# yondonfu/ai-rtc-agent

Hardware: NVIDIA H100
Metric: frames/sec at 512x512 SD-Turbo img2img (1-step, stream-batch 1) (higher is better)
Workload: dtype f16

## Files before the change

### ai-rtc-agent_b200/csrc/attention.cu

```cuda
#include "attention.cuh"

#include <cudaTypedefs.h>
#include <math.h>
#include <string.h>

#include "igemm.cuh"
#include "launch.cuh"
#include "ptx.cuh"
#include "wgmma.cuh"

namespace b2 {

constexpr int AT_BQ = 128;
constexpr int AT_STAGES = 3;
constexpr int AT_CONS = 256;
constexpr int AT_THREADS = AT_CONS + 32;

__device__ __forceinline__ float ex2_approx(float x) {
    float y;
    asm volatile("ex2.approx.ftz.f32 %0, %1;" : "=f"(y) : "f"(x));
    return y;
}

__device__ __forceinline__ uint32_t pack_half2(float a, float b) {
    const __half2 h = __floats2half2_rn(a, b);
    return *reinterpret_cast<const uint32_t*>(&h);
}

struct AttnParams {
    CUtensorMap tmq, tmk, tmv;
    __half* out;
    int ldo;
    int sq, skv, heads, d_real;
    long k_bstride, vt_bstride;
    float scale_log2;
};

struct AttnIpParams : AttnParams {
    CUtensorMap tmk_ip, tmv_ip;
    const int* n_ip;
};

template <int DA, int BKV, bool IP = false>
__global__ void __launch_bounds__(AT_THREADS, 1) attn_kernel(const __grid_constant__ std::conditional_t<IP, AttnIpParams, AttnParams> p) {
    constexpr int DP = DA * 64;
    constexpr int NST = AT_STAGES;
    constexpr int KVA = BKV / 64;
    constexpr uint32_t Q_BYTES = DA * AT_BQ * 128;
    constexpr uint32_t K_BYTES = DA * BKV * 128;
    constexpr uint32_t V_BYTES = KVA * DP * 128;
    constexpr uint32_t STAGE_BYTES = K_BYTES + V_BYTES;

    extern __shared__ __align__(1024) uint8_t smem[];
    uint8_t* sQ = smem;
    uint8_t* sKV = sQ + Q_BYTES;
    uint64_t* bars = reinterpret_cast<uint64_t*>(sKV + NST * STAGE_BYTES);
    uint64_t* q_full = bars;
    uint64_t* k_full = bars + 1;
    uint64_t* k_empty = k_full + NST;
    uint64_t* v_full = k_empty + NST;
    uint64_t* v_empty = v_full + NST;

    const int warp = threadIdx.x >> 5, lane = threadIdx.x & 31;
    const int q0 = blockIdx.x * AT_BQ;
    const int h = blockIdx.y, b = blockIdx.z;
    const int nblk = (p.skv + BKV - 1) / BKV;

    if (threadIdx.x == AT_CONS) {
        if (smem_u32(smem) & 1023u) {
            printf("b2 attn: dynamic smem base not 1024-aligned\n");
            __trap();
        }
        tma_prefetch_desc(&p.tmq);
        tma_prefetch_desc(&p.tmk);
        tma_prefetch_desc(&p.tmv);
        mbar_init(q_full, 1);
        for (int s = 0; s < NST; ++s) {
            mbar_init(&k_full[s], 1);
            mbar_init(&k_empty[s], AT_CONS / 32);
            mbar_init(&v_full[s], 1);
            mbar_init(&v_empty[s], AT_CONS / 32);
        }
        fence_mbar_init();
    }
    __syncthreads();
    pdl_launch_dependents();
    pdl_wait();
    int n_ip = 0;
    if constexpr (IP) n_ip = *p.n_ip;

    if (warp == AT_CONS / 32) {
        if (lane == 0) {
            mbar_expect_tx(q_full, Q_BYTES);
#pragma unroll
            for (int a = 0; a < DA; ++a)
                tma_load_2d(sQ + a * (AT_BQ * 128), &p.tmq, q_full, h * DP + a * 64, b * p.sq + q0);
            auto load_k = [&](int j) {
                const int st = j % NST;
                mbar_wait(&k_empty[st], ((j / NST) & 1) ^ 1);
                uint8_t* sk = sKV + st * STAGE_BYTES;
                mbar_expect_tx(&k_full[st], K_BYTES);
#pragma unroll
                for (int a = 0; a < DA; ++a)
                    tma_load_2d(sk + a * (BKV * 128), &p.tmk, &k_full[st], h * DP + a * 64, (int)(b * p.k_bstride) + j * BKV);
            };
            auto load_v = [&](int j) {
                const int st = j % NST;
                mbar_wait(&v_empty[st], ((j / NST) & 1) ^ 1);
                uint8_t* sv = sKV + st * STAGE_BYTES + K_BYTES;
                mbar_expect_tx(&v_full[st], V_BYTES);
#pragma unroll
                for (int a = 0; a < KVA; ++a)
                    tma_load_2d(sv + a * (DP * 128), &p.tmv, &v_full[st], (int)(b * p.vt_bstride) + j * BKV + a * 64, h * DP);
            };
            auto load_k_ip = [&]() {
                if constexpr (IP) {
                    const int st = nblk % NST;
                    mbar_wait(&k_empty[st], ((nblk / NST) & 1) ^ 1);
                    uint8_t* sk = sKV + st * STAGE_BYTES;
                    mbar_expect_tx(&k_full[st], DA * ATTN_IP_KEYS * 128);
#pragma unroll
                    for (int a = 0; a < DA; ++a)
                        tma_load_2d(sk + a * (ATTN_IP_KEYS * 128), &p.tmk_ip, &k_full[st], h * DP + a * 64, 0);
                }
            };
            auto load_v_ip = [&]() {
                if constexpr (IP) {
                    const int st = nblk % NST;
                    mbar_wait(&v_empty[st], ((nblk / NST) & 1) ^ 1);
                    mbar_expect_tx(&v_full[st], DP * 128);
                    tma_load_2d(sKV + st * STAGE_BYTES + K_BYTES, &p.tmv_ip, &v_full[st], 0, h * DP);
                }
            };
            load_k(0);
            for (int j = 0; j < nblk; ++j) {
                if (j + 1 < nblk) load_k(j + 1);
                else if (n_ip > 0) load_k_ip();
                load_v(j);
            }
            if (n_ip > 0) load_v_ip();
        }
    } else {
        const int wg = warp >> 2;
        const int rq = wg * 64 + (warp & 3) * 16 + (lane >> 2);
        const int q2 = 2 * (lane & 3);
        const uint32_t sq_addr = smem_u32(sQ) + (uint32_t)wg * (64 * 128), skv_addr = smem_u32(sKV);
        float m_run[2] = {-INFINITY, -INFINITY}, l_run[2] = {0.f, 0.f};
        float o[DP / 2];
#pragma unroll
        for (int i = 0; i < DP / 2; ++i) o[i] = 0.f;
        mbar_wait(q_full, 0);
        for (int j = 0; j < nblk; ++j) {
            const int st = j % NST;
            const uint32_t ph = (uint32_t)(j / NST) & 1u;
            const uint32_t sk = skv_addr + st * STAGE_BYTES;
            float s[BKV / 2];
#pragma unroll
            for (int i = 0; i < BKV / 2; ++i) s[i] = 0.f;
            mbar_wait(&k_full[st], ph);
            wgmma_fence_regs(s);
            wgmma_fence();
#pragma unroll
            for (int a = 0; a < DA; ++a) {
                const uint64_t dq = make_kmajor_sw128_desc(sq_addr + a * (AT_BQ * 128));
                const uint64_t dk = make_kmajor_sw128_desc(sk + a * (BKV * 128));
#pragma unroll
                for (int k = 0; k < 4; ++k) Wgmma<BKV>::ss(s, dq + 2 * k, dk + 2 * k, 1u);
            }
            wgmma_commit();
            wgmma_wait<0>();
            wgmma_fence_regs(s);
            if (lane == 0) mbar_arrive(&k_empty[st]);
            const int kv_valid = p.skv - j * BKV;
            float alpha[2], m_new[2];
#pragma unroll
            for (int hr = 0; hr < 2; ++hr) {
                float mx = -INFINITY;
#pragma unroll
                for (int jj = 0; jj < BKV / 8; ++jj)
#pragma unroll
                    for (int u = 0; u < 2; ++u)
                        if (8 * jj + q2 + u < kv_valid) mx = fmaxf(mx, s[4 * jj + 2 * hr + u]);
                mx = fmaxf(mx, __shfl_xor_sync(0xffffffffu, mx, 1));
                mx = fmaxf(mx, __shfl_xor_sync(0xffffffffu, mx, 2));
                m_new[hr] = fmaxf(m_run[hr], mx * p.scale_log2);
                alpha[hr] = ex2_approx(m_run[hr] - m_new[hr]);
            }
            uint32_t pa[BKV / 16][4];
            float rs[2] = {0.f, 0.f};
#pragma unroll
            for (int jj = 0; jj < BKV / 8; ++jj)
#pragma unroll
                for (int hr = 0; hr < 2; ++hr) {
                    float p0 = ex2_approx(s[4 * jj + 2 * hr] * p.scale_log2 - m_new[hr]);
                    float p1 = ex2_approx(s[4 * jj + 2 * hr + 1] * p.scale_log2 - m_new[hr]);
                    if (8 * jj + q2 >= kv_valid) p0 = 0.f;
                    if (8 * jj + q2 + 1 >= kv_valid) p1 = 0.f;
                    rs[hr] += p0 + p1;
                    pa[jj >> 1][(jj & 1) * 2 + hr] = pack_half2(p0, p1);
                }
#pragma unroll
            for (int hr = 0; hr < 2; ++hr) {
                l_run[hr] = l_run[hr] * alpha[hr] + rs[hr];
                m_run[hr] = m_new[hr];
            }
#pragma unroll
            for (int jj = 0; jj < DP / 8; ++jj)
#pragma unroll
                for (int hr = 0; hr < 2; ++hr) {
                    o[4 * jj + 2 * hr] *= alpha[hr];
                    o[4 * jj + 2 * hr + 1] *= alpha[hr];
                }
            const uint32_t sv = sk + K_BYTES;
            mbar_wait(&v_full[st], ph);
            wgmma_fence_regs(o);
            wgmma_fence();
#pragma unroll
            for (int kk = 0; kk < BKV / 16; ++kk) {
                const uint64_t dv = make_kmajor_sw128_desc(sv + (kk >> 2) * (DP * 128)) + 2 * (kk & 3);
                Wgmma<DP>::rs(o, pa[kk], dv, 1u);
            }
            wgmma_commit();
            wgmma_wait<0>();
            wgmma_fence_regs(o);
            if (lane == 0) mbar_arrive(&v_empty[st]);
        }
        if (n_ip > 0) {
            const int st = nblk % NST;
            const uint32_t ph = (uint32_t)(nblk / NST) & 1u;
            const uint32_t sk = skv_addr + st * STAGE_BYTES;
            float s[ATTN_IP_KEYS / 2];
#pragma unroll
            for (int i = 0; i < ATTN_IP_KEYS / 2; ++i) s[i] = 0.f;
            mbar_wait(&k_full[st], ph);
            wgmma_fence_regs(s);
            wgmma_fence();
#pragma unroll
            for (int a = 0; a < DA; ++a) {
                const uint64_t dq = make_kmajor_sw128_desc(sq_addr + a * (AT_BQ * 128));
                const uint64_t dk = make_kmajor_sw128_desc(sk + a * (ATTN_IP_KEYS * 128));
#pragma unroll
                for (int k = 0; k < 4; ++k) Wgmma<ATTN_IP_KEYS>::ss(s, dq + 2 * k, dk + 2 * k, 1u);
            }
            wgmma_commit();
            wgmma_wait<0>();
            wgmma_fence_regs(s);
            float m2[2], f2[2];
#pragma unroll
            for (int hr = 0; hr < 2; ++hr) {
                float mx = -INFINITY;
#pragma unroll
                for (int jj = 0; jj < ATTN_IP_KEYS / 8; ++jj)
#pragma unroll
                    for (int u = 0; u < 2; ++u)
                        if (8 * jj + q2 + u < n_ip) mx = fmaxf(mx, s[4 * jj + 2 * hr + u]);
                mx = fmaxf(mx, __shfl_xor_sync(0xffffffffu, mx, 1));
                mx = fmaxf(mx, __shfl_xor_sync(0xffffffffu, mx, 2));
                m2[hr] = mx * p.scale_log2;
            }
            float p2[ATTN_IP_KEYS / 2];
            float rs[2] = {0.f, 0.f};
#pragma unroll
            for (int jj = 0; jj < ATTN_IP_KEYS / 8; ++jj)
#pragma unroll
                for (int hr = 0; hr < 2; ++hr)
#pragma unroll
                    for (int u = 0; u < 2; ++u) {
                        float e = ex2_approx(s[4 * jj + 2 * hr + u] * p.scale_log2 - m2[hr]);
                        if (8 * jj + q2 + u >= n_ip) e = 0.f;
                        p2[4 * jj + 2 * hr + u] = e;
                        rs[hr] += e;
                    }
#pragma unroll
            for (int hr = 0; hr < 2; ++hr) {
                float l = l_run[hr], l2 = rs[hr];
                l += __shfl_xor_sync(0xffffffffu, l, 1);
                l += __shfl_xor_sync(0xffffffffu, l, 2);
                l2 += __shfl_xor_sync(0xffffffffu, l2, 1);
                l2 += __shfl_xor_sync(0xffffffffu, l2, 2);
                f2[hr] = l / l2;
            }
            uint32_t pa[ATTN_IP_KEYS / 16][4];
#pragma unroll
            for (int jj = 0; jj < ATTN_IP_KEYS / 8; ++jj)
#pragma unroll
                for (int hr = 0; hr < 2; ++hr)
                    pa[jj >> 1][(jj & 1) * 2 + hr] = pack_half2(p2[4 * jj + 2 * hr] * f2[hr], p2[4 * jj + 2 * hr + 1] * f2[hr]);
            const uint32_t sv = sk + K_BYTES;
            mbar_wait(&v_full[st], ph);
            wgmma_fence_regs(o);
            wgmma_fence();
#pragma unroll
            for (int kk = 0; kk < ATTN_IP_KEYS / 16; ++kk) Wgmma<DP>::rs(o, pa[kk], make_kmajor_sw128_desc(sv) + 2 * kk, 1u);
            wgmma_commit();
            wgmma_wait<0>();
            wgmma_fence_regs(o);
        }
#pragma unroll
        for (int hr = 0; hr < 2; ++hr) {
            float l = l_run[hr];
            l += __shfl_xor_sync(0xffffffffu, l, 1);
            l += __shfl_xor_sync(0xffffffffu, l, 2);
            const float inv_l = 1.0f / l;
            const int r = rq + 8 * hr;
            if (q0 + r >= p.sq) continue;
            __half* orow = p.out + ((long)b * p.sq + q0 + r) * p.ldo + h * p.d_real;
#pragma unroll
            for (int jj = 0; jj < DP / 8; ++jj) {
                const int col = 8 * jj + q2;
                if (col < p.d_real)
                    *reinterpret_cast<uint32_t*>(orow + col) = pack_half2(o[4 * jj + 2 * hr] * inv_l, o[4 * jj + 2 * hr + 1] * inv_l);
            }
        }
    }
}

constexpr int A5_D = 512;
constexpr int A5_DS = 128;
constexpr int A5_SLICES = A5_D / A5_DS;
constexpr int A5_BQ = 128;
constexpr int A5_BKV = 32;
constexpr int A5_THREADS = 256;
constexpr int A5_QP = A5_D + 8;
constexpr int A5_VP = A5_BKV + 8;
constexpr size_t A5_Q_ELEMS = (size_t)A5_BQ * A5_QP;
constexpr size_t A5_K_ELEMS = (size_t)A5_BKV * A5_QP;
constexpr size_t A5_V_ELEMS = (size_t)A5_DS * A5_VP;
constexpr size_t A5_SMEM = (A5_Q_ELEMS + 2 * (A5_K_ELEMS + A5_V_ELEMS)) * 2;

struct Attn512Params {
    const __half* q; const __half* k; const __half* vt;
    __half* out;
    int ldq, ldk, ldvt, ldo;
    int sq, skv;
    long k_bstride, vt_bstride;
    float scale_log2;
};

__device__ __forceinline__ void cp_async16(uint32_t dst, const void* src, int src_bytes) {
    asm volatile("cp.async.cg.shared.global [%0], [%1], 16, %2;" ::"r"(dst), "l"(src), "r"(src_bytes) : "memory");
}
__device__ __forceinline__ void cp_async_commit() { asm volatile("cp.async.commit_group;" ::: "memory"); }
template <int N>
__device__ __forceinline__ void cp_async_wait() { asm volatile("cp.async.wait_group %0;" ::"n"(N) : "memory"); }
__device__ __forceinline__ void ldsm_x4(uint32_t addr, uint32_t& r0, uint32_t& r1, uint32_t& r2, uint32_t& r3) {
    asm volatile("ldmatrix.sync.aligned.m8n8.x4.shared.b16 {%0,%1,%2,%3}, [%4];"
                 : "=r"(r0), "=r"(r1), "=r"(r2), "=r"(r3) : "r"(addr));
}
__device__ __forceinline__ void mma16816(float (&d)[4], const uint32_t (&a)[4], uint32_t b0, uint32_t b1) {
    asm volatile("mma.sync.aligned.m16n8k16.row.col.f32.f16.f16.f32 {%0,%1,%2,%3}, {%4,%5,%6,%7}, {%8,%9}, {%0,%1,%2,%3};"
                 : "+f"(d[0]), "+f"(d[1]), "+f"(d[2]), "+f"(d[3])
                 : "r"(a[0]), "r"(a[1]), "r"(a[2]), "r"(a[3]), "r"(b0), "r"(b1));
}

__global__ void __launch_bounds__(A5_THREADS, 1) attn_d512_kernel(const __grid_constant__ Attn512Params p) {
    extern __shared__ __align__(128) __half sm5[];
    __half* sQ = sm5;
    __half* sK = sQ + A5_Q_ELEMS;
    __half* sV = sK + 2 * A5_K_ELEMS;
    const int tid = threadIdx.x, warp = tid >> 5, lane = tid & 31;
    const int q0 = blockIdx.x * A5_BQ;
    const int head = blockIdx.y / A5_SLICES, slice = blockIdx.y % A5_SLICES;
    const int b = blockIdx.z;
    const int col0 = head * A5_D;
    const int nblk = (p.skv + A5_BKV - 1) / A5_BKV;
    const __half* qb = p.q + (long)b * p.sq * p.ldq + col0;
    const __half* kb = p.k + b * p.k_bstride * p.ldk + col0;
    const __half* vb = p.vt + (long)(col0 + slice * A5_DS) * p.ldvt + b * p.vt_bstride;

    pdl_launch_dependents();
    pdl_wait();

    for (int i = tid; i < A5_BQ * (A5_D / 8); i += A5_THREADS) {
        const int r = i / (A5_D / 8), c = (i % (A5_D / 8)) * 8;
        const bool ok = q0 + r < p.sq;
        cp_async16(smem_u32(sQ + r * A5_QP + c), ok ? qb + (long)(q0 + r) * p.ldq + c : qb, ok ? 16 : 0);
    }
    auto load_kv = [&](int j, int buf) {
        __half* sk = sK + buf * A5_K_ELEMS;
        __half* sv = sV + buf * A5_V_ELEMS;
        const int kv0 = j * A5_BKV;
        for (int i = tid; i < A5_BKV * (A5_D / 8); i += A5_THREADS) {
            const int r = i / (A5_D / 8), c = (i % (A5_D / 8)) * 8;
            const bool ok = kv0 + r < p.skv;
            cp_async16(smem_u32(sk + r * A5_QP + c), ok ? kb + (long)(kv0 + r) * p.ldk + c : kb, ok ? 16 : 0);
        }
        for (int i = tid; i < A5_DS * (A5_BKV / 8); i += A5_THREADS) {
            const int r = i / (A5_BKV / 8), c = (i % (A5_BKV / 8)) * 8;
            const int valid = p.skv - (kv0 + c);
            const int bytes = valid >= 8 ? 16 : (valid > 0 ? 2 * valid : 0);
            cp_async16(smem_u32(sv + r * A5_VP + c), bytes ? vb + (long)r * p.ldvt + kv0 + c : vb, bytes);
        }
    };
    load_kv(0, 0);
    cp_async_commit();

    const int r_lo = lane >> 2, q2 = 2 * (lane & 3);
    float o[A5_DS / 8][4];
#pragma unroll
    for (int n = 0; n < A5_DS / 8; ++n) o[n][0] = o[n][1] = o[n][2] = o[n][3] = 0.f;
    float m_run[2] = {-INFINITY, -INFINITY}, l_run[2] = {0.f, 0.f};
    const uint32_t a_base = smem_u32(sQ + (warp * 16 + (lane & 15)) * A5_QP + (lane >> 4) * 8);
    const int b_row = (lane & 7) + ((lane >> 4) << 3), b_col = ((lane >> 3) & 1) * 8;

    for (int j = 0; j < nblk; ++j) {
        const int buf = j & 1;
        if (j + 1 < nblk) {
            load_kv(j + 1, buf ^ 1);
            cp_async_commit();
            cp_async_wait<1>();
        } else {
            cp_async_wait<0>();
        }
        __syncthreads();
        float s[A5_BKV / 8][4];
#pragma unroll
        for (int n = 0; n < A5_BKV / 8; ++n) s[n][0] = s[n][1] = s[n][2] = s[n][3] = 0.f;
        const uint32_t k_base = smem_u32(sK + buf * A5_K_ELEMS + b_row * A5_QP + b_col);
#pragma unroll 4
        for (int kk = 0; kk < A5_D / 16; ++kk) {
            uint32_t a[4];
            ldsm_x4(a_base + kk * 32, a[0], a[1], a[2], a[3]);
#pragma unroll
            for (int np = 0; np < A5_BKV / 16; ++np) {
                uint32_t b0, b1, b2, b3;
                ldsm_x4(k_base + (np * 16 * A5_QP) * 2 + kk * 32, b0, b1, b2, b3);
                mma16816(s[2 * np], a, b0, b1);
                mma16816(s[2 * np + 1], a, b2, b3);
            }
        }
        const int kv_valid = p.skv - j * A5_BKV;
        float alpha[2], m_new[2];
#pragma unroll
        for (int hr = 0; hr < 2; ++hr) {
            float mx = -INFINITY;
#pragma unroll
            for (int n = 0; n < A5_BKV / 8; ++n)
#pragma unroll
                for (int u = 0; u < 2; ++u)
                    if (8 * n + q2 + u < kv_valid) mx = fmaxf(mx, s[n][2 * hr + u]);
            mx = fmaxf(mx, __shfl_xor_sync(0xffffffffu, mx, 1));
            mx = fmaxf(mx, __shfl_xor_sync(0xffffffffu, mx, 2));
            m_new[hr] = fmaxf(m_run[hr], mx * p.scale_log2);
            alpha[hr] = ex2_approx(m_run[hr] - m_new[hr]);
        }
        uint32_t pa[A5_BKV / 16][4];
        float rs[2] = {0.f, 0.f};
#pragma unroll
        for (int n = 0; n < A5_BKV / 8; ++n)
#pragma unroll
            for (int hr = 0; hr < 2; ++hr) {
                float p0 = ex2_approx(s[n][2 * hr] * p.scale_log2 - m_new[hr]);
                float p1 = ex2_approx(s[n][2 * hr + 1] * p.scale_log2 - m_new[hr]);
                if (8 * n + q2 >= kv_valid) p0 = 0.f;
                if (8 * n + q2 + 1 >= kv_valid) p1 = 0.f;
                rs[hr] += p0 + p1;
                pa[n >> 1][(n & 1) * 2 + hr] = pack_half2(p0, p1);
            }
#pragma unroll
        for (int hr = 0; hr < 2; ++hr) {
            l_run[hr] = l_run[hr] * alpha[hr] + rs[hr];
            m_run[hr] = m_new[hr];
        }
#pragma unroll
        for (int n = 0; n < A5_DS / 8; ++n) {
            o[n][0] *= alpha[0]; o[n][1] *= alpha[0];
            o[n][2] *= alpha[1]; o[n][3] *= alpha[1];
        }
        const uint32_t v_base = smem_u32(sV + buf * A5_V_ELEMS + b_row * A5_VP + b_col);
#pragma unroll
        for (int t = 0; t < A5_BKV / 16; ++t)
#pragma unroll
            for (int np = 0; np < A5_DS / 16; ++np) {
                uint32_t b0, b1, b2, b3;
                ldsm_x4(v_base + (np * 16 * A5_VP) * 2 + t * 32, b0, b1, b2, b3);
                mma16816(o[2 * np], pa[t], b0, b1);
                mma16816(o[2 * np + 1], pa[t], b2, b3);
            }
        __syncthreads();
    }
#pragma unroll
    for (int hr = 0; hr < 2; ++hr) {
        float l = l_run[hr];
        l += __shfl_xor_sync(0xffffffffu, l, 1);
        l += __shfl_xor_sync(0xffffffffu, l, 2);
        const float inv_l = 1.0f / l;
        const int r = q0 + warp * 16 + r_lo + 8 * hr;
        if (r >= p.sq) continue;
        __half* orow = p.out + ((long)b * p.sq + r) * p.ldo + col0 + slice * A5_DS;
#pragma unroll
        for (int n = 0; n < A5_DS / 8; ++n)
            *reinterpret_cast<uint32_t*>(orow + 8 * n + q2) = pack_half2(o[n][2 * hr] * inv_l, o[n][2 * hr + 1] * inv_l);
    }
}

static int encode_2d(CUtensorMap* m, const __half* ptr, long cols, long rows, long ld, int box_cols, int box_rows,
                     const char* what) {
    static PFN_cuTensorMapEncodeTiled_v12000 enc = nullptr;
    if (!enc) {
        void* fp = nullptr;
        cudaDriverEntryPointQueryResult qres;
        cudaError_t err = cudaGetDriverEntryPoint("cuTensorMapEncodeTiled", &fp, cudaEnableDefault, &qres);
        if (err != cudaSuccess || qres != cudaDriverEntryPointSuccess || !fp) {
            b2_set_error("cudaGetDriverEntryPoint(cuTensorMapEncodeTiled) failed");
            return -1;
        }
        enc = reinterpret_cast<PFN_cuTensorMapEncodeTiled_v12000>(fp);
    }
    cuuint64_t dims[2] = {(cuuint64_t)cols, (cuuint64_t)rows};
    cuuint64_t strides[1] = {(cuuint64_t)ld * 2};
    cuuint32_t box[2] = {(cuuint32_t)box_cols, (cuuint32_t)box_rows};
    cuuint32_t es[2] = {1, 1};
    CUresult r = enc(m, CU_TENSOR_MAP_DATA_TYPE_FLOAT16, 2, const_cast<__half*>(ptr), dims, strides, box, es,
                     CU_TENSOR_MAP_INTERLEAVE_NONE, CU_TENSOR_MAP_SWIZZLE_128B, CU_TENSOR_MAP_L2_PROMOTION_L2_256B,
                     CU_TENSOR_MAP_FLOAT_OOB_FILL_NONE);
    if (r != CUDA_SUCCESS) {
        b2_set_error("attn: cuTensorMapEncodeTiled(%s) failed: %d (cols %ld rows %ld ld %ld box %d,%d)", what, (int)r,
                     cols, rows, ld, box_cols, box_rows);
        return -1;
    }
    return 0;
}

static size_t attn_smem_bytes(int da, int bkv) {
    const size_t q = (size_t)da * AT_BQ * 128;
    const size_t k = (size_t)da * bkv * 128;
    const size_t v = (size_t)(bkv / 64) * da * 64 * 128;
    return q + AT_STAGES * (k + v) + 256;
}

int attn_plan(const AttnDesc& d, AttnPlan* plan) {
    *plan = AttnPlan{};
    if (d.dp == A5_D) {
        const auto misaligned = [](const void* ptr) { return (reinterpret_cast<uintptr_t>(ptr) & 15) != 0; };
        if (d.d_real != A5_D || (d.ldq & 7) || (d.ldk & 7) || (d.ldvt & 7) || (d.ldo & 7) || (d.vt_bstride & 7) ||
            misaligned(d.q) || misaligned(d.k) || misaligned(d.vt) || misaligned(d.out) || d.sq < 1 || d.skv < 1) {
            b2_set_error("attn(d512): needs d_real 512, row pitches and the V^T batch stride multiples of 8, 16-byte aligned "
                         "pointers (d_real %d ldq %d ldk %d ldvt %d ldo %d vt_bstride %ld)", d.d_real, d.ldq, d.ldk, d.ldvt, d.ldo,
                         d.vt_bstride);
            return -1;
        }
        plan->d = d;
        plan->grid = dim3((d.sq + A5_BQ - 1) / A5_BQ, d.heads * A5_SLICES, d.nb);
        plan->smem = A5_SMEM;
        return 0;
    }
    if (d.dp != 64 && d.dp != 128 && d.dp != 192) {
        b2_set_error("attn: padded head dim %d unsupported", d.dp);
        return -1;
    }
    if (d.d_real > d.dp || (d.d_real & 7) || (d.ldo & 7) || (d.ldq & 7) || (d.ldk & 7) || (d.ldvt & 7)) {
        b2_set_error("attn: bad dims d_real %d dp %d", d.d_real, d.dp);
        return -1;
    }
    plan->d = d;
    const int bkv = (d.dp == 192) ? 64 : 128;
    if (encode_2d(&plan->tmq, d.q, (long)d.heads * d.dp, (long)d.nb * d.sq, d.ldq, 64, AT_BQ, "q")) return -1;
    if (encode_2d(&plan->tmk, d.k, (long)d.heads * d.dp, d.k_rows, d.ldk, 64, bkv, "k")) return -1;
    if (encode_2d(&plan->tmv, d.vt, d.vt_cols, (long)d.heads * d.dp, d.ldvt, 64, d.dp, "vt")) return -1;
    if (d.n_ip || d.k_ip || d.vt_ip) {
        const auto misaligned = [](const void* ptr) { return (reinterpret_cast<uintptr_t>(ptr) & 15) != 0; };
        if (!d.n_ip || !d.k_ip || !d.vt_ip || misaligned(d.k_ip) || misaligned(d.vt_ip)) {
            b2_set_error("attn: the image segment needs k_ip, vt_ip (16-byte aligned) and n_ip together");
            return -1;
        }
        if (encode_2d(&plan->tmk_ip, d.k_ip, (long)d.heads * d.dp, ATTN_IP_KEYS, d.ldk, 64, ATTN_IP_KEYS, "k_ip")) return -1;
        if (encode_2d(&plan->tmv_ip, d.vt_ip, ATTN_IP_KEYS, (long)d.heads * d.dp, ATTN_IP_KEYS, 64, d.dp, "vt_ip")) return -1;
    }
    plan->grid = dim3((d.sq + AT_BQ - 1) / AT_BQ, d.heads, d.nb);
    plan->smem = attn_smem_bytes(d.dp / 64, bkv);
    return 0;
}

static const void* attn_ip_kernel(int dp) {
    return dp == 64 ? (const void*)attn_kernel<1, 128, true>
                    : dp == 128 ? (const void*)attn_kernel<2, 128, true> : (const void*)attn_kernel<3, 64, true>;
}

int attn_init() {
    static bool attr_set = false;
    if (!attr_set) {
        cudaError_t e1 = cudaFuncSetAttribute(attn_kernel<1, 128>, cudaFuncAttributeMaxDynamicSharedMemorySize, 227 * 1024);
        cudaError_t e2 = cudaFuncSetAttribute(attn_kernel<2, 128>, cudaFuncAttributeMaxDynamicSharedMemorySize, 227 * 1024);
        cudaError_t e3 = cudaFuncSetAttribute(attn_kernel<3, 64>, cudaFuncAttributeMaxDynamicSharedMemorySize, 227 * 1024);
        cudaError_t e4 = cudaFuncSetAttribute(attn_d512_kernel, cudaFuncAttributeMaxDynamicSharedMemorySize, (int)A5_SMEM);
        if (e1 != cudaSuccess || e2 != cudaSuccess || e3 != cudaSuccess || e4 != cudaSuccess) {
            b2_set_error("cudaFuncSetAttribute(attn) failed");
            return -1;
        }
        for (int dp : {64, 128, 192})
            if (cudaFuncSetAttribute(attn_ip_kernel(dp), cudaFuncAttributeMaxDynamicSharedMemorySize, 227 * 1024) != cudaSuccess) {
                b2_set_error("cudaFuncSetAttribute(attn, image segment) failed");
                return -1;
            }
        attr_set = true;
    }
    return 0;
}

int attn_launch(const AttnPlan& plan, cudaStream_t s) {
    if (attn_init()) return -1;
    const AttnDesc& d = plan.d;
    if (d.dp == A5_D) {
        Attn512Params q5;
        q5.q = d.q; q5.k = d.k; q5.vt = d.vt; q5.out = d.out;
        q5.ldq = d.ldq; q5.ldk = d.ldk; q5.ldvt = d.ldvt; q5.ldo = d.ldo;
        q5.sq = d.sq; q5.skv = d.skv; q5.k_bstride = d.k_bstride; q5.vt_bstride = d.vt_bstride;
        q5.scale_log2 = (float)(1.4426950408889634 / sqrt((double)d.d_real));
        const cudaError_t e5 = launch_k(attn_d512_kernel, plan.grid, dim3(A5_THREADS), plan.smem, s, 1, q5);
        if (e5 != cudaSuccess) {
            b2_set_error("attn(d512) launch: %s", cudaGetErrorString(e5));
            return -1;
        }
        return 0;
    }
    AttnParams p;
    p.tmq = plan.tmq; p.tmk = plan.tmk; p.tmv = plan.tmv;
    p.out = d.out; p.ldo = d.ldo;
    p.sq = d.sq; p.skv = d.skv; p.heads = d.heads; p.d_real = d.d_real;
    p.k_bstride = d.k_bstride; p.vt_bstride = d.vt_bstride;
    p.scale_log2 = (float)(1.4426950408889634 / sqrt((double)d.d_real));
    cudaError_t e;
    if (d.n_ip) {
        AttnIpParams pi;
        static_cast<AttnParams&>(pi) = p;
        pi.tmk_ip = plan.tmk_ip; pi.tmv_ip = plan.tmv_ip;
        pi.n_ip = d.n_ip;
        if (d.dp == 64) e = launch_k(attn_kernel<1, 128, true>, plan.grid, dim3(AT_THREADS), plan.smem, s, 1, pi);
        else if (d.dp == 128) e = launch_k(attn_kernel<2, 128, true>, plan.grid, dim3(AT_THREADS), plan.smem, s, 1, pi);
        else e = launch_k(attn_kernel<3, 64, true>, plan.grid, dim3(AT_THREADS), plan.smem, s, 1, pi);
    } else if (d.dp == 64) e = launch_k(attn_kernel<1, 128>, plan.grid, dim3(AT_THREADS), plan.smem, s, 1, p);
    else if (d.dp == 128) e = launch_k(attn_kernel<2, 128>, plan.grid, dim3(AT_THREADS), plan.smem, s, 1, p);
    else e = launch_k(attn_kernel<3, 64>, plan.grid, dim3(AT_THREADS), plan.smem, s, 1, p);
    if (e != cudaSuccess) {
        b2_set_error("attn launch: %s", cudaGetErrorString(e));
        return -1;
    }
    return 0;
}

}
```

### ai-rtc-agent_b200/csrc/ptx.cuh

```cuda
#pragma once
#include <cuda.h>
#include <cuda_fp16.h>
#include <cuda_runtime.h>
#include <stdint.h>
#include <stdio.h>

namespace b2 {

__device__ __forceinline__ uint32_t smem_u32(const void* p) {
    return static_cast<uint32_t>(__cvta_generic_to_shared(p));
}

__device__ __forceinline__ uint64_t globaltimer_ns() {
    uint64_t t;
    asm volatile("mov.u64 %0, %%globaltimer;" : "=l"(t));
    return t;
}

__device__ __forceinline__ void mbar_init(uint64_t* bar, uint32_t count) {
    asm volatile("mbarrier.init.shared::cta.b64 [%0], %1;" ::"r"(smem_u32(bar)), "r"(count));
}
__device__ __forceinline__ void fence_mbar_init() {
    asm volatile("fence.mbarrier_init.release.cluster;" ::: "memory");
}
__device__ __forceinline__ void mbar_expect_tx(uint64_t* bar, uint32_t bytes) {
    asm volatile("mbarrier.arrive.expect_tx.shared::cta.b64 _, [%0], %1;" ::"r"(smem_u32(bar)),
                 "r"(bytes)
                 : "memory");
}
__device__ __forceinline__ void mbar_arrive(uint64_t* bar) {
    asm volatile("mbarrier.arrive.shared::cta.b64 _, [%0];" ::"r"(smem_u32(bar)) : "memory");
}
__device__ __forceinline__ bool mbar_try_wait(uint64_t* bar, uint32_t parity) {
    uint32_t ok;
    asm volatile(
        "{\n\t"
        ".reg .pred P;\n\t"
        "mbarrier.try_wait.parity.shared::cta.b64 P, [%1], %2;\n\t"
        "selp.u32 %0, 1, 0, P;\n\t"
        "}\n"
        : "=r"(ok)
        : "r"(smem_u32(bar)), "r"(parity)
        : "memory");
    return ok != 0;
}
#ifndef B2_WAIT_TIMEOUT_NS
#define B2_WAIT_TIMEOUT_NS 4000000000ull
#endif
__device__ __forceinline__ void mbar_wait(uint64_t* bar, uint32_t parity) {
    if (mbar_try_wait(bar, parity)) return;
    uint64_t t0 = 0;
    uint32_t spins = 0;
    while (!mbar_try_wait(bar, parity)) {
        if ((++spins & 0x3ff) == 0) {
            const uint64_t now = globaltimer_ns();
            if (t0 == 0) t0 = now;
            else if (now - t0 > B2_WAIT_TIMEOUT_NS) __trap();
        }
    }
}

__device__ __forceinline__ void mbar_arrive_remote(uint32_t cluster_addr) {
    asm volatile("mbarrier.arrive.shared::cluster.b64 _, [%0];" ::"r"(cluster_addr) : "memory");
}

__device__ __forceinline__ void fence_proxy_async_smem() {
    asm volatile("fence.proxy.async.shared::cta;" ::: "memory");
}

__device__ __forceinline__ void cluster_sync_all() {
    asm volatile("barrier.cluster.arrive.release.aligned;" ::: "memory");
    asm volatile("barrier.cluster.wait.acquire.aligned;" ::: "memory");
}
__device__ __forceinline__ void cluster_arrive_relaxed() { asm volatile("barrier.cluster.arrive.relaxed.aligned;" ::: "memory"); }
__device__ __forceinline__ void cluster_wait() { asm volatile("barrier.cluster.wait.aligned;" ::: "memory"); }
__device__ __forceinline__ uint32_t cluster_ctarank() {
    uint32_t r;
    asm volatile("mov.u32 %0, %%cluster_ctarank;" : "=r"(r));
    return r;
}
__device__ __forceinline__ uint32_t dsmem_map(uint32_t local_smem_addr, uint32_t rank) {
    uint32_t r;
    asm volatile("mapa.shared::cluster.u32 %0, %1, %2;" : "=r"(r) : "r"(local_smem_addr), "r"(rank));
    return r;
}
__device__ __forceinline__ void dsmem_st_f2(uint32_t cluster_addr, float x, float y) {
    asm volatile("st.shared::cluster.v2.f32 [%0], {%1, %2};" ::"r"(cluster_addr), "f"(x), "f"(y) : "memory");
}
__device__ __forceinline__ float4 dsmem_ld_f4(uint32_t cluster_addr) {
    float4 v;
    asm volatile("ld.shared::cluster.v4.f32 {%0, %1, %2, %3}, [%4];"
                 : "=f"(v.x), "=f"(v.y), "=f"(v.z), "=f"(v.w)
                 : "r"(cluster_addr)
                 : "memory");
    return v;
}

__device__ __forceinline__ void tma_prefetch_desc(const CUtensorMap* m) {
    asm volatile("prefetch.tensormap [%0];" ::"l"(reinterpret_cast<uint64_t>(m)) : "memory");
}
__device__ __forceinline__ void tma_load_2d(void* smem_dst, const CUtensorMap* m, uint64_t* bar,
                                            int c0, int c1) {
    asm volatile(
        "cp.async.bulk.tensor.2d.shared::cluster.global.mbarrier::complete_tx::bytes [%0], [%1, {%3, "
        "%4}], [%2];" ::"r"(smem_u32(smem_dst)),
        "l"(reinterpret_cast<uint64_t>(m)), "r"(smem_u32(bar)), "r"(c0), "r"(c1)
        : "memory");
}
__device__ __forceinline__ void tma_load_4d(void* smem_dst, const CUtensorMap* m, uint64_t* bar,
                                            int c0, int c1, int c2, int c3) {
    asm volatile(
        "cp.async.bulk.tensor.4d.shared::cluster.global.mbarrier::complete_tx::bytes [%0], [%1, {%3, "
        "%4, %5, %6}], [%2];" ::"r"(smem_u32(smem_dst)),
        "l"(reinterpret_cast<uint64_t>(m)), "r"(smem_u32(bar)), "r"(c0), "r"(c1), "r"(c2), "r"(c3)
        : "memory");
}

__device__ __forceinline__ void tma_store_4d(const CUtensorMap* m, const void* smem_src, int c0, int c1, int c2, int c3) {
    asm volatile("cp.async.bulk.tensor.4d.global.shared::cta.bulk_group [%0, {%2, %3, %4, %5}], [%1];" ::"l"(reinterpret_cast<uint64_t>(m)),
                 "r"(smem_u32(smem_src)), "r"(c0), "r"(c1), "r"(c2), "r"(c3)
                 : "memory");
}
__device__ __forceinline__ void bulk_commit_group() { asm volatile("cp.async.bulk.commit_group;" ::: "memory"); }
template <int N>
__device__ __forceinline__ void bulk_wait_group_read() { asm volatile("cp.async.bulk.wait_group.read %0;" ::"n"(N) : "memory"); }
template <int N>
__device__ __forceinline__ void bulk_wait_group() { asm volatile("cp.async.bulk.wait_group %0;" ::"n"(N) : "memory"); }

__device__ __forceinline__ void named_bar_sync(int id, int count) {
    asm volatile("bar.sync %0, %1;" ::"r"(id), "r"(count) : "memory");
}

__device__ __forceinline__ void tma_load_2d_mc(void* smem_dst, const CUtensorMap* m, uint64_t* bar, int c0, int c1, uint16_t cta_mask) {
    asm volatile(
        "cp.async.bulk.tensor.2d.shared::cluster.global.mbarrier::complete_tx::bytes.multicast::cluster [%0], [%1, {%3, %4}], [%2], "
        "%5;" ::"r"(smem_u32(smem_dst)),
        "l"(reinterpret_cast<uint64_t>(m)), "r"(smem_u32(bar)), "r"(c0), "r"(c1), "h"(cta_mask)
        : "memory");
}

__device__ __forceinline__ void wgmma_fence() { asm volatile("wgmma.fence.sync.aligned;" ::: "memory"); }
__device__ __forceinline__ void wgmma_commit() { asm volatile("wgmma.commit_group.sync.aligned;" ::: "memory"); }
template <int N>
__device__ __forceinline__ void wgmma_wait() { asm volatile("wgmma.wait_group.sync.aligned %0;" ::"n"(N) : "memory"); }
template <int N>
__device__ __forceinline__ void wgmma_fence_regs(float (&d)[N]) {
#pragma unroll
    for (int i = 0; i < N; ++i) asm volatile("" : "+f"(d[i])::"memory");
}

__device__ __forceinline__ uint64_t make_kmajor_sw128_desc(uint32_t smem_addr, uint32_t sbo = 1024) {
    uint64_t d = 0;
    d |= (uint64_t)((smem_addr & 0x3ffff) >> 4);
    d |= (uint64_t)1 << 16;
    d |= (uint64_t)(sbo >> 4) << 32;
    d |= (uint64_t)1 << 62;
    return d;
}

}
```

Measured before the change: 199.9.

## Add warpgroup ping-pong and QK/PV overlap to flash attention kernel

Expands the producer to a full warpgroup so setmaxnreg can move registers from the TMA producer to the consumer warpgroups. Two consumer warpgroups alternate tensor-core issue through named barriers (ping-pong), so one group's softmax overlaps the other's MMA. For head dim 64 it also pipelines QK of block j with PV of block j-1 within a warpgroup. Masking is split so full KV blocks skip per-element bounds checks. The risks are more threads per block, register pressure at the 240-register cap, and barrier-ordering subtleties.

```diff
diff --git a/ai-rtc-agent_b200/csrc/attention.cu b/ai-rtc-agent_b200/csrc/attention.cu
--- a/ai-rtc-agent_b200/csrc/attention.cu
+++ b/ai-rtc-agent_b200/csrc/attention.cu
@@ -14,7 +14,10 @@
 constexpr int AT_BQ = 128;
 constexpr int AT_STAGES = 3;
 constexpr int AT_CONS = 256;
-constexpr int AT_THREADS = AT_CONS + 32;
+constexpr int AT_THREADS = AT_CONS + 128;
+constexpr int AT_PROD_REGS = 24, AT_CONS_REGS = 240;
+template <int DA>
+constexpr bool AT_OVERLAP = DA == 1;
 
 __device__ __forceinline__ float ex2_approx(float x) {
     float y;
@@ -25,6 +28,43 @@
 __device__ __forceinline__ uint32_t pack_half2(float a, float b) {
     const __half2 h = __floats2half2_rn(a, b);
     return *reinterpret_cast<const uint32_t*>(&h);
+}
+
+template <int BKV, bool MASK>
+__device__ __forceinline__ void attn_softmax(float (&s)[BKV / 2], int kv_valid, int q2, float scale_log2, float (&m_run)[2],
+                                             float (&l_run)[2], float (&alpha)[2]) {
+    float m_new[2];
+#pragma unroll
+    for (int hr = 0; hr < 2; ++hr) {
+        float mx = -INFINITY;
+#pragma unroll
+        for (int jj = 0; jj < BKV / 8; ++jj)
+#pragma unroll
+            for (int u = 0; u < 2; ++u)
+                if (!MASK || 8 * jj + q2 + u < kv_valid) mx = fmaxf(mx, s[4 * jj + 2 * hr + u]);
+        mx = fmaxf(mx, __shfl_xor_sync(0xffffffffu, mx, 1));
+        mx = fmaxf(mx, __shfl_xor_sync(0xffffffffu, mx, 2));
+        m_new[hr] = fmaxf(m_run[hr], mx * scale_log2);
+        alpha[hr] = ex2_approx(m_run[hr] - m_new[hr]);
+    }
+    float rs[2] = {0.f, 0.f};
+#pragma unroll
+    for (int jj = 0; jj < BKV / 8; ++jj)
+#pragma unroll
+        for (int hr = 0; hr < 2; ++hr) {
+            float p0 = ex2_approx(s[4 * jj + 2 * hr] * scale_log2 - m_new[hr]);
+            float p1 = ex2_approx(s[4 * jj + 2 * hr + 1] * scale_log2 - m_new[hr]);
+            if (MASK && 8 * jj + q2 >= kv_valid) p0 = 0.f;
+            if (MASK && 8 * jj + q2 + 1 >= kv_valid) p1 = 0.f;
+            rs[hr] += p0 + p1;
+            s[4 * jj + 2 * hr] = p0;
+            s[4 * jj + 2 * hr + 1] = p1;
+        }
+#pragma unroll
+    for (int hr = 0; hr < 2; ++hr) {
+        l_run[hr] = l_run[hr] * alpha[hr] + rs[hr];
+        m_run[hr] = m_new[hr];
+    }
 }
 
 struct AttnParams {
@@ -86,11 +126,14 @@
     __syncthreads();
     pdl_launch_dependents();
     pdl_wait();
-    int n_ip = 0;
-    if constexpr (IP) n_ip = *p.n_ip;
-
-    if (warp == AT_CONS / 32) {
-        if (lane == 0) {
+    const auto image_keys = [&]() -> int {
+        if constexpr (IP) return *p.n_ip;
+        else return 0;
+    };
+
+    if (warp >= AT_CONS / 32) {
+        setmaxnreg_dec<AT_PROD_REGS>();
+        if (warp == AT_CONS / 32 && lane == 0) {
             mbar_expect_tx(q_full, Q_BYTES);
 #pragma unroll
             for (int a = 0; a < DA; ++a)
@@ -132,6 +175,7 @@
                     tma_load_2d(sKV + st * STAGE_BYTES + K_BYTES, &p.tmv_ip, &v_full[st], 0, h * DP);
                 }
             };
+            const int n_ip = image_keys();
             load_k(0);
             for (int j = 0; j < nblk; ++j) {
                 if (j + 1 < nblk) load_k(j + 1);
@@ -141,6 +185,7 @@
             if (n_ip > 0) load_v_ip();
         }
     } else {
+        setmaxnreg_inc<AT_CONS_REGS>();
         const int wg = warp >> 2;
         const int rq = wg * 64 + (warp & 3) * 16 + (lane >> 2);
         const int q2 = 2 * (lane & 3);
@@ -150,81 +195,108 @@
 #pragma unroll
         for (int i = 0; i < DP / 2; ++i) o[i] = 0.f;
         mbar_wait(q_full, 0);
-        for (int j = 0; j < nblk; ++j) {
-            const int st = j % NST;
-            const uint32_t ph = (uint32_t)(j / NST) & 1u;
-            const uint32_t sk = skv_addr + st * STAGE_BYTES;
+        if (nblk > 0) {
+            const int my_turn = 1 + wg, next_turn = 2 - wg;
+            if (wg == 1) named_bar_arrive(1, AT_CONS);
             float s[BKV / 2];
-#pragma unroll
-            for (int i = 0; i < BKV / 2; ++i) s[i] = 0.f;
-            mbar_wait(&k_full[st], ph);
-            wgmma_fence_regs(s);
-            wgmma_fence();
-#pragma unroll
-            for (int a = 0; a < DA; ++a) {
-                const uint64_t dq = make_kmajor_sw128_desc(sq_addr + a * (AT_BQ * 128));
-                const uint64_t dk = make_kmajor_sw128_desc(sk + a * (BKV * 128));
-#pragma unroll
-                for (int k = 0; k < 4; ++k) Wgmma<BKV>::ss(s, dq + 2 * k, dk + 2 * k, 1u);
-            }
-            wgmma_commit();
-            wgmma_wait<0>();
-            wgmma_fence_regs(s);
-            if (lane == 0) mbar_arrive(&k_empty[st]);
-            const int kv_valid = p.skv - j * BKV;
-            float alpha[2], m_new[2];
-#pragma unroll
-            for (int hr = 0; hr < 2; ++hr) {
-                float mx = -INFINITY;
+            uint32_t pa[BKV / 16][4];
+            float alpha[2];
+            auto issue_qk = [&](int j) {
+                const uint32_t sk = skv_addr + (j % NST) * STAGE_BYTES;
+#pragma unroll
+                for (int i = 0; i < BKV / 2; ++i) s[i] = 0.f;
+                wgmma_fence_regs(s);
+                wgmma_fence_regs(o);
+                wgmma_fence();
+#pragma unroll
+                for (int a = 0; a < DA; ++a) {
+                    const uint64_t dq = make_kmajor_sw128_desc(sq_addr + a * (AT_BQ * 128));
+                    const uint64_t dk = make_kmajor_sw128_desc(sk + a * (BKV * 128));
+#pragma unroll
+                    for (int k = 0; k < 4; ++k) Wgmma<BKV>::ss(s, dq + 2 * k, dk + 2 * k, 1u);
+                }
+                wgmma_commit();
+            };
+            auto issue_pv = [&](int j) {
+                const uint32_t sv = skv_addr + (j % NST) * STAGE_BYTES + K_BYTES;
+#pragma unroll
+                for (int kk = 0; kk < BKV / 16; ++kk) {
+                    const uint64_t dv = make_kmajor_sw128_desc(sv + (kk >> 2) * (DP * 128)) + 2 * (kk & 3);
+                    Wgmma<DP>::rs(o, pa[kk], dv, 1u);
+                }
+            };
+            auto softmax = [&](int j) {
+                if ((j + 1) * BKV <= p.skv) attn_softmax<BKV, false>(s, BKV, q2, p.scale_log2, m_run, l_run, alpha);
+                else attn_softmax<BKV, true>(s, p.skv - j * BKV, q2, p.scale_log2, m_run, l_run, alpha);
+            };
+            auto rescale_pack = [&]() {
+#pragma unroll
+                for (int jj = 0; jj < DP / 8; ++jj)
+#pragma unroll
+                    for (int hr = 0; hr < 2; ++hr) {
+                        o[4 * jj + 2 * hr] *= alpha[hr];
+                        o[4 * jj + 2 * hr + 1] *= alpha[hr];
+                    }
 #pragma unroll
                 for (int jj = 0; jj < BKV / 8; ++jj)
 #pragma unroll
-                    for (int u = 0; u < 2; ++u)
-                        if (8 * jj + q2 + u < kv_valid) mx = fmaxf(mx, s[4 * jj + 2 * hr + u]);
-                mx = fmaxf(mx, __shfl_xor_sync(0xffffffffu, mx, 1));
-                mx = fmaxf(mx, __shfl_xor_sync(0xffffffffu, mx, 2));
-                m_new[hr] = fmaxf(m_run[hr], mx * p.scale_log2);
-                alpha[hr] = ex2_approx(m_run[hr] - m_new[hr]);
-            }
-            uint32_t pa[BKV / 16][4];
-            float rs[2] = {0.f, 0.f};
-#pragma unroll
-            for (int jj = 0; jj < BKV / 8; ++jj)
-#pragma unroll
-                for (int hr = 0; hr < 2; ++hr) {
-                    float p0 = ex2_approx(s[4 * jj + 2 * hr] * p.scale_log2 - m_new[hr]);
-                    float p1 = ex2_approx(s[4 * jj + 2 * hr + 1] * p.scale_log2 - m_new[hr]);
-                    if (8 * jj + q2 >= kv_valid) p0 = 0.f;
-                    if (8 * jj + q2 + 1 >= kv_valid) p1 = 0.f;
-                    rs[hr] += p0 + p1;
-                    pa[jj >> 1][(jj & 1) * 2 + hr] = pack_half2(p0, p1);
+                    for (int hr = 0; hr < 2; ++hr)
+                        pa[jj >> 1][(jj & 1) * 2 + hr] = pack_half2(s[4 * jj + 2 * hr], s[4 * jj + 2 * hr + 1]);
+            };
+            auto k_phase = [](int j) { return (uint32_t)(j / NST) & 1u; };
+            if constexpr (AT_OVERLAP<DA>) {
+                for (int j = 0; j < nblk; ++j) {
+                    mbar_wait(&k_full[j % NST], k_phase(j));
+                    if (j > 0) mbar_wait(&v_full[(j - 1) % NST], k_phase(j - 1));
+                    named_bar_sync(my_turn, AT_CONS);
+                    issue_qk(j);
+                    if (j > 0) issue_pv(j - 1);
+                    wgmma_commit();
+                    named_bar_arrive(next_turn, AT_CONS);
+                    wgmma_wait<1>();
+                    wgmma_fence_regs(s);
+                    if (lane == 0) mbar_arrive(&k_empty[j % NST]);
+                    softmax(j);
+                    wgmma_wait<0>();
+                    wgmma_fence_regs(o);
+                    if (j > 0 && lane == 0) mbar_arrive(&v_empty[(j - 1) % NST]);
+                    rescale_pack();
                 }
-#pragma unroll
-            for (int hr = 0; hr < 2; ++hr) {
-                l_run[hr] = l_run[hr] * alpha[hr] + rs[hr];
-                m_run[hr] = m_new[hr];
-            }
-#pragma unroll
-            for (int jj = 0; jj < DP / 8; ++jj)
-#pragma unroll
-                for (int hr = 0; hr < 2; ++hr) {
-                    o[4 * jj + 2 * hr] *= alpha[hr];
-                    o[4 * jj + 2 * hr + 1] *= alpha[hr];
+                mbar_wait(&v_full[(nblk - 1) % NST], k_phase(nblk - 1));
+                named_bar_sync(my_turn, AT_CONS);
+                wgmma_fence_regs(o);
+                wgmma_fence();
+                issue_pv(nblk - 1);
+                wgmma_commit();
+                if (wg == 0) named_bar_arrive(next_turn, AT_CONS);
+                wgmma_wait<0>();
+                wgmma_fence_regs(o);
+                if (lane == 0) mbar_arrive(&v_empty[(nblk - 1) % NST]);
+            } else {
+                for (int j = 0; j < nblk; ++j) {
+                    mbar_wait(&k_full[j % NST], k_phase(j));
+                    named_bar_sync(my_turn, AT_CONS);
+                    issue_qk(j);
+                    named_bar_arrive(next_turn, AT_CONS);
+                    wgmma_wait<0>();
+                    wgmma_fence_regs(s);
+                    if (lane == 0) mbar_arrive(&k_empty[j % NST]);
+                    softmax(j);
+                    rescale_pack();
+                    mbar_wait(&v_full[j % NST], k_phase(j));
+                    named_bar_sync(my_turn, AT_CONS);
+                    wgmma_fence_regs(o);
+                    wgmma_fence();
+                    issue_pv(j);
+                    wgmma_commit();
+                    if (wg == 0 || j + 1 < nblk) named_bar_arrive(next_turn, AT_CONS);
+                    wgmma_wait<0>();
+                    wgmma_fence_regs(o);
+                    if (lane == 0) mbar_arrive(&v_empty[j % NST]);
                 }
-            const uint32_t sv = sk + K_BYTES;
-            mbar_wait(&v_full[st], ph);
-            wgmma_fence_regs(o);
-            wgmma_fence();
-#pragma unroll
-            for (int kk = 0; kk < BKV / 16; ++kk) {
-                const uint64_t dv = make_kmajor_sw128_desc(sv + (kk >> 2) * (DP * 128)) + 2 * (kk & 3);
-                Wgmma<DP>::rs(o, pa[kk], dv, 1u);
-            }
-            wgmma_commit();
-            wgmma_wait<0>();
-            wgmma_fence_regs(o);
-            if (lane == 0) mbar_arrive(&v_empty[st]);
-        }
+            }
+        }
+        const int n_ip = image_keys();
         if (n_ip > 0) {
             const int st = nblk % NST;
             const uint32_t ph = (uint32_t)(nblk / NST) & 1u;
diff --git a/ai-rtc-agent_b200/csrc/ptx.cuh b/ai-rtc-agent_b200/csrc/ptx.cuh
--- a/ai-rtc-agent_b200/csrc/ptx.cuh
+++ b/ai-rtc-agent_b200/csrc/ptx.cuh
@@ -130,6 +130,14 @@
 __device__ __forceinline__ void named_bar_sync(int id, int count) {
     asm volatile("bar.sync %0, %1;" ::"r"(id), "r"(count) : "memory");
 }
+__device__ __forceinline__ void named_bar_arrive(int id, int count) {
+    asm volatile("bar.arrive %0, %1;" ::"r"(id), "r"(count) : "memory");
+}
+
+template <uint32_t N>
+__device__ __forceinline__ void setmaxnreg_dec() { asm volatile("setmaxnreg.dec.sync.aligned.u32 %0;" ::"n"(N)); }
+template <uint32_t N>
+__device__ __forceinline__ void setmaxnreg_inc() { asm volatile("setmaxnreg.inc.sync.aligned.u32 %0;" ::"n"(N)); }
 
 __device__ __forceinline__ void tma_load_2d_mc(void* smem_dst, const CUtensorMap* m, uint64_t* bar, int c0, int c1, uint16_t cta_mask) {
     asm volatile(
```

After: 201.8, median of 6. About the same (+0.9%).
